# pdh930105/ARCQuant

Hardware: AMD Instinct MI355X
Metric: ARC-NVFP4 GEMM TFLOP/s (M=4096, N=KQ=4096, KE=64) (higher is better)
Workload: dtype f16

## Files before the change

### arcquant_amd/csrc/gemm_tile.hip

```cpp
#include <hip/hip_runtime.h>
#include <stdint.h>
#include <stdlib.h>

#include <type_traits>

#include "arcq_internal.hpp"
#include "gemm_common.hpp"
#include "gemm_tile_common.hpp"

namespace arcq {

#ifdef ARCQ_STREAM_STAMPS
static unsigned long long* g_tile_stamps = nullptr;
extern "C" void arcq_debug_set_tile_stamps(void* p) { g_tile_stamps = reinterpret_cast<unsigned long long*>(p); }
#define ARCQ_TILE_STAMP(k)                                                                                     \
  do {                                                                                                         \
    if (p.stamps && tid == 0) {                                                                                \
      unsigned long long t0_, t1_;                                                                             \
      asm volatile("s_memtime %0\n\ts_memrealtime %1\n\ts_waitcnt lgkmcnt(0)" : "=s"(t0_), "=s"(t1_)::"memory"); \
      p.stamps[(size_t)blockIdx.x * 4 + 2 * (k)] = t0_;                                                        \
      p.stamps[(size_t)blockIdx.x * 4 + 2 * (k) + 1] = t1_;                                                    \
    }                                                                                                          \
  } while (0)
#else
#define ARCQ_TILE_STAMP(k) do { } while (0)
#endif

template <int BM, int BN, int WAVES_M, int WAVES_N, bool kMfma32, int kEpi, bool kStagger, bool kPipe>
__global__ __launch_bounds__(WAVES_M* WAVES_N * 64) void gemm_tile_kernel(TileParams p) {
  constexpr int kThreads = WAVES_M * WAVES_N * 64;
  constexpr int WM = BM / WAVES_M, WN = BN / WAVES_N;
  constexpr int kT = kMfma32 ? 32 : 16;
  constexpr int TM = WM / kT, TN = WN / kT;
  using acc_t = typename std::conditional<kMfma32, f32x16, f32x4>::type;
  constexpr int A_UNITS = (BM * 2 + kThreads - 1) / kThreads, B_UNITS = (BN * 2 + kThreads - 1) / kThreads;
  constexpr bool A_PARTIAL = (BM * 2) % kThreads != 0, B_PARTIAL = (BN * 2) % kThreads != 0;
  static_assert(!A_PARTIAL || A_UNITS == 1, "a partial A pass is a single pass");
  static_assert(!B_PARTIAL || B_UNITS == 1, "a partial B pass is a single pass");
  constexpr int A_TILE = BM * kRowBytes, B_TILE = BN * kRowBytes;

  extern __shared__ __attribute__((aligned(16))) unsigned char smem[];
  unsigned char* const lds_a0 = smem;
  unsigned char* const lds_b0 = smem + A_TILE;
  unsigned char* const lds_a1 = smem + A_TILE + B_TILE;
  unsigned char* const lds_b1 = smem + 2 * A_TILE + B_TILE;

  const int ntiles = p.tiles_m * p.tiles_n;
  int bid = blockIdx.x, split = 0;
  if (p.splits > 1) {
    split = bid / ntiles;
    bid -= split * ntiles;
  }
  {
    const int q8 = ntiles >> 3, r8 = ntiles & 7, x = bid & 7, j = bid >> 3;
    bid = (x < r8 ? x * (q8 + 1) : r8 * (q8 + 1) + (x - r8) * q8) + j;
  }
  constexpr int kGroupM = 8;
  const int per_group = kGroupM * p.tiles_n;
  const int grp = bid / per_group;
  const int first_m = grp * kGroupM;
  const int gsz = min(p.tiles_m - first_m, kGroupM);
  const int tm = first_m + (bid % per_group) % gsz;
  const int tn = (bid % per_group) / gsz;
  const int m0 = tm * BM, n0 = tn * BN;

  const int tid = threadIdx.x;
  const int lane = tid & 63, wave = tid >> 6;
  const int wr = wave / WAVES_N, wc = wave % WAVES_N;
  const int half_k = p.K >> 1, atoms_k = p.K >> 6;
  const int a_begin = split * p.atoms_per_split, a_end = min(atoms_k, a_begin + p.atoms_per_split);

  const uint8_t* a_q[A_UNITS];
  const uint8_t* a_sf[A_UNITS];
  uint32_t a_live[A_UNITS];
  int a_slot[A_UNITS][4];
#pragma unroll
  for (int u = 0; u < A_UNITS; ++u) {
    const int unit = tid + u * kThreads, r = A_PARTIAL ? min(unit >> 1, BM - 1) : unit >> 1, h = unit & 1;
    const int row = m0 + r, rc = row < p.M ? row : p.M - 1;
    a_q[u] = p.A + (size_t)rc * half_k + h * 16;
    a_sf[u] = p.SFA + sf_atom_offset(rc, 0, atoms_k) + h * 2;
    a_live[u] = row < p.M ? 0xffffu : 0u;
#pragma unroll
    for (int j = 0; j < 4; ++j) a_slot[u][j] = kMfma32 ? lds_slot32(r, h * 4 + j) : lds_slot(r, h * 4 + j);
  }
  const uint8_t* b_q[B_UNITS];
  const uint8_t* b_sf[B_UNITS];
  uint32_t b_live[B_UNITS];
  int b_slot[B_UNITS][4];
#pragma unroll
  for (int u = 0; u < B_UNITS; ++u) {
    const int unit = tid + u * kThreads, r = B_PARTIAL ? min(unit >> 1, BN - 1) : unit >> 1, h = unit & 1;
    const int row = n0 + r, rc = row < p.N ? row : p.N - 1;
    b_q[u] = p.B + (size_t)rc * half_k + h * 16;
    b_sf[u] = p.SFB + sf_atom_offset(rc, 0, atoms_k) + h * 2;
    b_live[u] = row < p.N ? 0xffffu : 0u;
#pragma unroll
    for (int j = 0; j < 4; ++j) b_slot[u][j] = kMfma32 ? lds_slot32(r, h * 4 + j) : lds_slot(r, h * 4 + j);
  }
  const int fa_base = kMfma32 ? lds_slot32(wr * WM + (lane & 31), lane >> 5) : lds_slot(wr * WM + (lane & 15), lane >> 4);
  const int fb_base = kMfma32 ? lds_slot32(wc * WN + (lane & 31), lane >> 5) : lds_slot(wc * WN + (lane & 15), lane >> 4);
  acc_t acc[TM][TN];
#pragma unroll
  for (int i = 0; i < TM; ++i)
#pragma unroll
    for (int j = 0; j < TN; ++j)
#pragma unroll
      for (int r = 0; r < (kMfma32 ? 16 : 4); ++r) acc[i][j][r] = 0.f;

  Staged sa[A_UNITS], sb[B_UNITS];
  auto load_step = [&](int atom) {
#pragma unroll
    for (int u = 0; u < A_UNITS; ++u) sa[u] = stage_load(a_q[u], a_sf[u], atom);
#pragma unroll
    for (int u = 0; u < B_UNITS; ++u) sb[u] = stage_load(b_q[u], b_sf[u], atom);
  };
  auto store_step = [&](unsigned char* la, unsigned char* lb) {
#pragma unroll
    for (int u = 0; u < A_UNITS; ++u)
      if (!A_PARTIAL || tid < BM * 2) stage_store(la, a_slot[u], sa[u], a_live[u]);
#pragma unroll
    for (int u = 0; u < B_UNITS; ++u)
      if (!B_PARTIAL || tid < BN * 2) stage_store(lb, b_slot[u], sb[u], b_live[u]);
  };
  auto mma_step = [&](const unsigned char* la, const unsigned char* lb) {
    if constexpr (kMfma32) {
#pragma unroll
      for (int ks = 0; ks < 4; ++ks) {
        Frag8 fa[TM], fb[TN];
#pragma unroll
        for (int i = 0; i < TM; ++i) fa[i].u = *reinterpret_cast<const uint4*>(la + (fa_base ^ (ks * 32)) + i * 32 * kRowBytes);
#pragma unroll
        for (int j = 0; j < TN; ++j) fb[j].u = *reinterpret_cast<const uint4*>(lb + (fb_base ^ (ks * 32)) + j * 32 * kRowBytes);
#pragma unroll
        for (int i = 0; i < TM; ++i)
#pragma unroll
          for (int j = 0; j < TN; ++j) acc[i][j] = __builtin_amdgcn_mfma_f32_32x32x16_f16(fb[j].v, fa[i].v, acc[i][j], 0, 0, 0);
      }
    } else {
#pragma unroll
      for (int ks = 0; ks < 2; ++ks) {
        Frag8 fa[TM], fb[TN];
#pragma unroll
        for (int i = 0; i < TM; ++i) fa[i].u = *reinterpret_cast<const uint4*>(la + (fa_base ^ (ks * 64)) + i * 16 * kRowBytes);
#pragma unroll
        for (int j = 0; j < TN; ++j) fb[j].u = *reinterpret_cast<const uint4*>(lb + (fb_base ^ (ks * 64)) + j * 16 * kRowBytes);
#pragma unroll
        for (int i = 0; i < TM; ++i)
#pragma unroll
          for (int j = 0; j < TN; ++j) acc[i][j] = __builtin_amdgcn_mfma_f32_16x16x32_f16(fb[j].v, fa[i].v, acc[i][j], 0, 0, 0);
      }
    }
  };
  const bool late = kStagger && wave >= 4;
  auto k_step = [&](int kt, unsigned char* ca, unsigned char* cb, unsigned char* na, unsigned char* nb) {
    Staged ta[A_UNITS], tb[B_UNITS];
#pragma unroll
    for (int u = 0; u < A_UNITS; ++u) ta[u] = sa[u];
#pragma unroll
    for (int u = 0; u < B_UNITS; ++u) tb[u] = sb[u];
    load_step(min(kt + 2 + (late ? 1 : 0), a_end - 1));
    __builtin_amdgcn_sched_barrier(0);
    mma_step(ca, cb);
    if (kStagger && late) __syncthreads();
    unsigned char* const wa = late ? ca : na;
    unsigned char* const wb = late ? cb : nb;
#pragma unroll
    for (int u = 0; u < A_UNITS; ++u)
      if (!A_PARTIAL || tid < BM * 2) stage_store(wa, a_slot[u], ta[u], a_live[u]);
#pragma unroll
    for (int u = 0; u < B_UNITS; ++u)
      if (!B_PARTIAL || tid < BN * 2) stage_store(wb, b_slot[u], tb[u], b_live[u]);
    if (!kStagger || !late) __syncthreads();
  };

  auto k_step_pipe = [&](int kt, unsigned char* ca, unsigned char* cb, unsigned char* na, unsigned char* nb) {
    static_assert(kMfma32 || TM % 2 == 0, "pairs of A fragments");
    Staged ta[A_UNITS], tb[B_UNITS];
#pragma unroll
    for (int u = 0; u < A_UNITS; ++u) ta[u] = sa[u];
#pragma unroll
    for (int u = 0; u < B_UNITS; ++u) tb[u] = sb[u];
    load_step(min(kt + 2, a_end - 1));
    __builtin_amdgcn_sched_barrier(0);
    constexpr int kPieces = (A_UNITS + B_UNITS) * 4, kBlocks = kMfma32 ? 4 : TM;
    auto pieces = [&](int blk) {
#pragma unroll
      for (int c = blk; c < kPieces; c += kBlocks) {
        const int u = c >> 2, j = c & 3;
        if (u < A_UNITS) {
#ifdef ARCQ_EXPERIMENT_A_RAW
          if (!A_PARTIAL || tid < BM * 2) stage_piece_raw(na, a_slot[u < A_UNITS ? u : 0][j], ta[u < A_UNITS ? u : 0], a_live[u < A_UNITS ? u : 0], j);
#else
          if (!A_PARTIAL || tid < BM * 2) stage_piece(na, a_slot[u < A_UNITS ? u : 0][j], ta[u < A_UNITS ? u : 0], a_live[u < A_UNITS ? u : 0], j);
#endif
        } else {
          const int v = u - A_UNITS < B_UNITS ? u - A_UNITS : 0;
#ifdef ARCQ_EXPERIMENT_B_RAW
          if (!B_PARTIAL || tid < BN * 2) stage_piece_raw(nb, b_slot[v][j], tb[v], b_live[v], j);
#else
          if (!B_PARTIAL || tid < BN * 2) stage_piece(nb, b_slot[v][j], tb[v], b_live[v], j);
#endif
        }
      }
    };
    if constexpr (kMfma32) {
      Frag8 f32a[2][TM], f32b[2][TN];
      auto rd_set = [&](int buf, int ks) {
#pragma unroll
        for (int i = 0; i < TM; ++i) f32a[buf][i].u = *reinterpret_cast<const uint4*>(ca + (fa_base ^ (ks * 32)) + i * 32 * kRowBytes);
#pragma unroll
        for (int j = 0; j < TN; ++j) f32b[buf][j].u = *reinterpret_cast<const uint4*>(cb + (fb_base ^ (ks * 32)) + j * 32 * kRowBytes);
      };
      rd_set(0, 0);
#pragma unroll
      for (int ks = 0; ks < 4; ++ks) {
        if (ks + 1 < 4) rd_set((ks + 1) & 1, ks + 1);
        __builtin_amdgcn_sched_barrier(0);
#pragma unroll
        for (int i = 0; i < TM; ++i)
#pragma unroll
          for (int j = 0; j < TN; ++j)
            if constexpr (kMfma32)
              acc[i][j] = __builtin_amdgcn_mfma_f32_32x32x16_f16(f32b[ks & 1][j].v, f32a[ks & 1][i].v, acc[i][j], 0, 0, 0);
        pieces(ks);
        __builtin_amdgcn_sched_barrier(0);
      }
      __syncthreads();
      return;
    }
    auto rd_a = [&](int ks, int i) { Frag8 f; f.u = *reinterpret_cast<const uint4*>(ca + (fa_base ^ (ks * 64)) + i * 16 * kRowBytes); return f; };
    auto rd_b = [&](int ks, int j) { Frag8 f; f.u = *reinterpret_cast<const uint4*>(cb + (fb_base ^ (ks * 64)) + j * 16 * kRowBytes); return f; };
    constexpr int kPairs = TM / 2, kSeq = 2 * kPairs, kAhead = 1;
    Frag8 fb[2][TN], fq[kSeq][2];
    auto rd_pair = [&](int q) {
      fq[q][0] = rd_a(q / kPairs, 2 * (q % kPairs));
      fq[q][1] = rd_a(q / kPairs, 2 * (q % kPairs) + 1);
    };
#pragma unroll
    for (int j = 0; j < TN; ++j) fb[0][j] = rd_b(0, j);
#pragma unroll
    for (int q = 0; q < kAhead; ++q) rd_pair(q);
#pragma unroll
    for (int q = 0; q < kSeq; ++q) {
      const int ks = q / kPairs, pr = q % kPairs;
      if (q + kAhead < kSeq) rd_pair(q + kAhead);
      if (ks == 0 && pr == kPairs - 1 - (kAhead - 1 < kPairs - 1 ? kAhead - 1 : kPairs - 1)) {
#pragma unroll
        for (int j = 0; j < TN; ++j) fb[1][j] = rd_b(1, j);
      }
      __builtin_amdgcn_sched_barrier(0);
#pragma unroll
      for (int ii = 0; ii < 2; ++ii)
#pragma unroll
        for (int j = 0; j < TN; ++j)
          if constexpr (!kMfma32)
            acc[2 * pr + ii][j] = __builtin_amdgcn_mfma_f32_16x16x32_f16(fb[ks][j].v, fq[q][ii].v, acc[2 * pr + ii][j], 0, 0, 0);
      pieces(q);
#pragma unroll
      for (int m8 = 0; m8 < (TM == 8 ? 2 * TN : 0); ++m8) {
        __builtin_amdgcn_sched_group_barrier(0x008, 1, 0);
        __builtin_amdgcn_sched_group_barrier(0x002, 2, 0);
      }
      __builtin_amdgcn_sched_barrier(0);
    }
    __syncthreads();
  };

  load_step(a_begin);
  store_step(lds_a0, lds_b0);
  load_step(min(a_begin + 1, a_end - 1));
  if (kStagger && late) {
    store_step(lds_a1, lds_b1);
    load_step(min(a_begin + 2, a_end - 1));
  }
  __syncthreads();
  int kt = a_begin;
  if (WAVES_M * WAVES_N == 8 && wave >= 4) __builtin_amdgcn_s_setprio(1);
  ARCQ_TILE_STAMP(0);
  if constexpr (kPipe) {
    for (; kt + 1 < a_end; kt += 2) {
      k_step_pipe(kt, lds_a0, lds_b0, lds_a1, lds_b1);
      k_step_pipe(kt + 1, lds_a1, lds_b1, lds_a0, lds_b0);
    }
    if (kt < a_end) k_step_pipe(kt, lds_a0, lds_b0, lds_a1, lds_b1);
  } else {
    for (; kt + 1 < a_end; kt += 2) {
      k_step(kt, lds_a0, lds_b0, lds_a1, lds_b1);
      k_step(kt + 1, lds_a1, lds_b1, lds_a0, lds_b0);
    }
    if (kt < a_end) k_step(kt, lds_a0, lds_b0, lds_a1, lds_b1);
  }
  ARCQ_TILE_STAMP(1);

  const float alpha = p.alpha_host * (p.alpha_dev ? *p.alpha_dev : 1.0f);
  const bool vec_ok = (p.N & 3) == 0;
  uint32_t act_max = 0;
  auto store4 = [&](int m, int n, float d0, float d1, float d2, float d3, bool pre, uint2 bias2, uint2 res2) __attribute__((always_inline)) {
    if (m >= p.M || n >= p.N) return;
    const uint32_t bw[2] = {bias2.x, bias2.y}, rw[2] = {res2.x, res2.y};
    auto bias_at = [&](int r) { return bf16_bits_to_f32(pre ? (bw[r >> 1] >> (16 * (r & 1))) & 0xffffu : (uint32_t)p.bias[n + r]); };
    if (kEpi == kEpiSiluMul) {
      uint32_t y[4] = {f32_to_bf16_bits(alpha * d0), f32_to_bf16_bits(alpha * d1), f32_to_bf16_bits(alpha * d2), f32_to_bf16_bits(alpha * d3)};
      if (p.bias) {
#pragma unroll
        for (int e = 0; e < 4; ++e) y[e] = f32_to_bf16_bits(bf16_bits_to_f32(y[e]) + bias_at(e));
      }
      const uint32_t a0 = silu_mul_bf16(y[0], y[1]);
      const uint32_t a1 = silu_mul_bf16(y[2], y[3]);
      *reinterpret_cast<uint32_t*>(reinterpret_cast<uint16_t*>(p.D) + (size_t)m * (p.N >> 1) + (n >> 1)) = a0 | (a1 << 16);
      act_max = max(act_max, max(a0 & 0x7fffu, a1 & 0x7fffu));
      return;
    }
    if (p.splits > 1) {
      *reinterpret_cast<float4*>(p.partial + ((size_t)split * p.M + m) * p.N + n) = make_float4(d0, d1, d2, d3);
      return;
    }
    float d[4] = {alpha * d0, alpha * d1, alpha * d2, alpha * d3};
    if (p.bias) {
#pragma unroll
      for (int r = 0; r < 4; ++r)
        if (pre || n + r < p.N) d[r] = (p.out_dtype == ARCQ_OUT_F32 ? d[r] : bf16_bits_to_f32(f32_to_bf16_bits(d[r]))) + bias_at(r);
    }
    if (p.residual) {
#pragma unroll
      for (int r = 0; r < 4; ++r)
        if (pre || n + r < p.N) {
          const float res = bf16_bits_to_f32(pre ? (rw[r >> 1] >> (16 * (r & 1))) & 0xffffu : (uint32_t)p.residual[(size_t)m * p.N + n + r]);
          d[r] = (p.out_dtype == ARCQ_OUT_F32 ? d[r] : bf16_bits_to_f32(f32_to_bf16_bits(d[r]))) + res;
        }
    }
    if (p.out_dtype == ARCQ_OUT_F32) {
      float* o = reinterpret_cast<float*>(p.D) + (size_t)m * p.N + n;
      if (vec_ok) *reinterpret_cast<float4*>(o) = make_float4(d[0], d[1], d[2], d[3]);
      else for (int r = 0; r < 4; ++r) if (n + r < p.N) o[r] = d[r];
    } else {
      uint16_t* o = reinterpret_cast<uint16_t*>(p.D) + (size_t)m * p.N + n;
      if (vec_ok) *reinterpret_cast<uint2*>(o) = make_uint2(pack_bf16x2(d[0], d[1]), pack_bf16x2(d[2], d[3]));
      else for (int r = 0; r < 4; ++r) if (n + r < p.N) o[r] = (uint16_t)f32_to_bf16_bits(d[r]);
    }
  };
  if constexpr (kMfma32) {
#pragma unroll
    for (int i = 0; i < TM; ++i)
#pragma unroll
      for (int j = 0; j < TN; ++j) {
        const int m = m0 + wr * WM + i * 32 + (lane & 31);
#pragma unroll
        for (int g = 0; g < 4; ++g) {
          const int n = n0 + wc * WN + j * 32 + 8 * g + 4 * (lane >> 5);
          store4(m, n, acc[i][j][4 * g + 0], acc[i][j][4 * g + 1], acc[i][j][4 * g + 2], acc[i][j][4 * g + 3], false, make_uint2(0, 0), make_uint2(0, 0));
        }
      }
  } else {
    const bool pre = vec_ok && p.splits <= 1 && ((reinterpret_cast<uintptr_t>(p.bias) | reinterpret_cast<uintptr_t>(p.residual)) & 7) == 0;
    const int nb = n0 + wc * WN + 4 * (lane >> 4), mb = m0 + wr * WM + (lane & 15);
    if (pre) {
      uint2 bias_v[TN], res_cur[TN], res_nxt[TN];
#pragma unroll
      for (int j = 0; j < TN; ++j) {
        bias_v[j] = res_cur[j] = res_nxt[j] = make_uint2(0, 0);
        if (p.bias && nb + j * 16 < p.N) bias_v[j] = *reinterpret_cast<const uint2*>(p.bias + nb + j * 16);
      }
      auto res_load = [&](int i, uint2 (&r)[TN]) {
        if (!p.residual) return;
        const int m = mb + i * 16;
#pragma unroll
        for (int j = 0; j < TN; ++j)
          if (m < p.M && nb + j * 16 < p.N) r[j] = *reinterpret_cast<const uint2*>(p.residual + (size_t)m * p.N + nb + j * 16);
      };
      res_load(0, res_cur);
#pragma unroll
      for (int i = 0; i < TM; ++i) {
        if (i + 1 < TM) res_load(i + 1, res_nxt);
#pragma unroll
        for (int j = 0; j < TN; ++j) store4(mb + i * 16, nb + j * 16, acc[i][j][0], acc[i][j][1], acc[i][j][2], acc[i][j][3], true, bias_v[j], res_cur[j]);
#pragma unroll
        for (int j = 0; j < TN; ++j) res_cur[j] = res_nxt[j];
      }
    } else {
#pragma unroll
      for (int i = 0; i < TM; ++i)
#pragma unroll
        for (int j = 0; j < TN; ++j)
          store4(mb + i * 16, nb + j * 16, acc[i][j][0], acc[i][j][1], acc[i][j][2], acc[i][j][3], false, make_uint2(0, 0), make_uint2(0, 0));
    }
  }
  if (kEpi == kEpiSiluMul) {
    __shared__ uint32_t wave_max[WAVES_M * WAVES_N];
#pragma unroll
    for (int sh = 32; sh > 0; sh >>= 1) act_max = max(act_max, (uint32_t)__shfl_down((int)act_max, sh, 64));
    if (lane == 0) wave_max[wave] = act_max;
    __syncthreads();
    if (tid == 0) {
      uint32_t m = 0;
#pragma unroll
      for (int w = 0; w < WAVES_M * WAVES_N; ++w) m = max(m, wave_max[w]);
      p.slots[blockIdx.x] = m;
    }
  }
}

struct TileCfg { int id, bm, bn, waves; };
static constexpr TileCfg kTileCfgs[] = {{1, 128, 128, 4}, {2, 256, 256, 4}, {3, 256, 256, 8}, {4, 128, 256, 4}, {5, 256, 256, 8}, {6, 128, 128, 4},
                                        {7, 64, 256, 4}, {8, 32, 256, 4}, {9, 128, 128, 4}, {10, 128, 256, 8}, {11, 256, 128, 8}, {12, 128, 128, 8},
                                        {13, 64, 256, 8}, {14, 64, 128, 8}, {15, 64, 64, 4}, {16, 64, 128, 4}, {17, 128, 64, 4}};
static const TileCfg& tile_cfg(int id) {
  for (const TileCfg& c : kTileCfgs)
    if (c.id == id) return c;
  return kTileCfgs[2];
}

static int env_int(const char* name, int dflt) {
  const char* e = getenv(name);
  return e ? atoi(e) : dflt;
}
static int tile_cfg_override() {
  static const int v = env_int("ARCQ_TILE_CFG", 0);
  return v;
}
static int tile_split_override() {
  static const int v = env_int("ARCQ_TILE_SPLIT", 0);
  return v;
}
static bool tile_stagger() {
  static const int v = env_int("ARCQ_TILE_STAGGER", 0);
  return v != 0;
}
static bool tile_pipe() {
  static const int v = env_int("ARCQ_TILE_PIPE", 1);
  return v != 0;
}

static void tile_split(int64_t M, int64_t N, int64_t K, int BM, int BN, int* splits, int* atoms_per_split) {
  const int64_t tiles = ((M + BM - 1) / BM) * ((N + BN - 1) / BN);
  const int atoms = (int)(K / 64);
  int s = 1;
  if ((N % 4) == 0) {
    if (tile_split_override() > 0) s = min(tile_split_override(), max(atoms / 2, 1));
    else
      while (tiles * s < 256 && atoms / (s * 2) >= 8 && s < 32) s *= 2;
  }
  const int per = (atoms + s - 1) / s;
  *splits = (atoms + per - 1) / per;
  *atoms_per_split = per;
}

template <int BM, int BN, int WAVES_M, int WAVES_N, bool kMfma32 = false, int kEpi = kEpiPlain>
static int launch_tile(const GemmArgs& a, hipStream_t stream, bool allow_split = false) {
  TileParams p;
  p.A = a.A; p.B = a.B; p.SFA = a.SFA; p.SFB = a.SFB; p.D = a.D;
  p.alpha_dev = a.alpha_dev; p.bias = a.bias; p.residual = a.residual;
  p.M = a.M; p.N = a.N; p.K = a.K; p.alpha_host = a.alpha_host; p.out_dtype = a.out_dtype;
  p.tiles_m = (a.M + BM - 1) / BM;
  p.tiles_n = (a.N + BN - 1) / BN;
  p.splits = 1; p.atoms_per_split = a.K / 64; p.partial = nullptr;
  p.epi = a.epilogue; p.slots = a.absmax_slots;
#ifdef ARCQ_STREAM_STAMPS
  p.stamps = g_tile_stamps;
#endif
  if (allow_split && a.epilogue == kEpiPlain) {
    tile_split(a.M, a.N, a.K, BM, BN, &p.splits, &p.atoms_per_split);
    if (p.splits > 1) {
      const int64_t need = (int64_t)p.splits * a.M * a.N * (int64_t)sizeof(float);
      if (!a.workspace || a.workspace_bytes < need)
        return fail(ARCQ_ERR_WORKSPACE, "arcq_gemm_nvfp4: split-K needs %lld B of workspace, got %lld", (long long)need,
                    (long long)a.workspace_bytes);
      p.partial = reinterpret_cast<float*>(a.workspace);
    }
  }
  const size_t lds = 2 * (size_t)(BM + BN) * kRowBytes;
  constexpr bool kCanStagger = WAVES_M * WAVES_N == 8 && BM == 256 && BN == 256, kCanPipe = true;
  auto kern = gemm_tile_kernel<BM, BN, WAVES_M, WAVES_N, kMfma32, kEpi, false, false>;
  if (kCanPipe && tile_pipe()) kern = gemm_tile_kernel<BM, BN, WAVES_M, WAVES_N, kMfma32, kEpi, false, kCanPipe>;
  else if (kCanStagger && tile_stagger()) kern = gemm_tile_kernel<BM, BN, WAVES_M, WAVES_N, kMfma32, kEpi, kCanStagger, false>;
  static LdsOptIn lds_opt[3];
  const int which = (kCanPipe && tile_pipe()) ? 1 : (kCanStagger && tile_stagger()) ? 2 : 0;
  if (int rc = ensure_dynamic_lds(reinterpret_cast<const void*>(kern), lds_opt[which], (int)lds, "arcq_gemm_nvfp4 (tile)")) return rc;
  hipLaunchKernelGGL(kern, dim3((unsigned)(p.tiles_m * p.tiles_n * p.splits)), dim3(WAVES_M * WAVES_N * 64), lds, stream, p);
  hipError_t e = hipGetLastError();
  if (e != hipSuccess) return fail(ARCQ_ERR_LAUNCH, "arcq_gemm_nvfp4 (tile): launch failed: %s", hipGetErrorString(e));
  if (p.splits > 1) return gemm_splitk_finish(a, p.splits, stream);
  return ARCQ_OK;
}

static int tile_choice(int64_t M, int64_t N, int64_t K) {
  const int64_t t256 = ((M + 255) / 256) * ((N + 255) / 256);
  if (t256 >= 192) return 3;
  if (M <= 32) return 8;
  if (M <= 64) return 7;
  const int64_t t10 = ((M + 127) / 128) * ((N + 255) / 256);
  if (t10 <= 64 || t10 == 128 || (t10 > 224 && t10 <= 256) || (K >= 8192 && t10 >= 96 && t10 <= 256)) return 10;
  return 1;
}

static int effective_cfg(int64_t M, int64_t N, int64_t K, bool* may_split) {
  int id = tile_cfg_override();
  if (id == 0) id = tile_choice(M, N, K);
  id = tile_cfg(id).id;
  *may_split = !(id >= 2 && id <= 6) && id != 9;
  return id;
}

int64_t gemm_tile_silu_slots(int64_t M, int64_t N, int64_t K) {
  bool sp;
  const TileCfg& c = tile_cfg(effective_cfg(M, N, K, &sp));
  return ((M + c.bm - 1) / c.bm) * ((N + c.bn - 1) / c.bn);
}

int64_t gemm_tile_workspace_bytes(int64_t M, int64_t N, int64_t K) {
  int s = 1, per = 0;
  bool sp;
  const TileCfg& c = tile_cfg(effective_cfg(M, N, K, &sp));
  if (sp) tile_split(M, N, K, c.bm, c.bn, &s, &per);
  return s > 1 ? (int64_t)s * M * N * (int64_t)sizeof(float) : 0;
}

template <int kEpi>
static int gemm_tile_epi(const GemmArgs& a, hipStream_t stream) {
  bool sp;
  switch (effective_cfg(a.M, a.N, a.K, &sp)) {
    case 1: case 9: return launch_tile<128, 128, 2, 2, false, kEpi>(a, stream, sp);
    case 2: return launch_tile<256, 256, 2, 2, false, kEpi>(a, stream);
    case 4: return launch_tile<128, 256, 2, 2, false, kEpi>(a, stream);
    case 5: return launch_tile<256, 256, 2, 4, true, kEpi>(a, stream);
    case 6: return launch_tile<128, 128, 2, 2, true, kEpi>(a, stream);
    case 7: return launch_tile<64, 256, 1, 4, false, kEpi>(a, stream, sp);
    case 8: return launch_tile<32, 256, 1, 4, false, kEpi>(a, stream, sp);
    case 10: return launch_tile<128, 256, 2, 4, false, kEpi>(a, stream, sp);
    case 11: return launch_tile<256, 128, 4, 2, false, kEpi>(a, stream, sp);
    case 12: return launch_tile<128, 128, 2, 4, false, kEpi>(a, stream, sp);
    case 13: return launch_tile<64, 256, 1, 8, false, kEpi>(a, stream, sp);
    case 14: return launch_tile<64, 128, 2, 4, false, kEpi>(a, stream, sp);
    case 15: return launch_tile<64, 64, 2, 2, false, kEpi>(a, stream, sp);
    case 16: return launch_tile<64, 128, 2, 2, false, kEpi>(a, stream, sp);
    case 17: return launch_tile<128, 64, 2, 2, false, kEpi>(a, stream, sp);
    default: return launch_tile<256, 256, 2, 4, false, kEpi>(a, stream);
  }
}

int gemm_tile(const GemmArgs& a, hipStream_t stream) {
  return a.epilogue == kEpiSiluMul ? gemm_tile_epi<kEpiSiluMul>(a, stream) : gemm_tile_epi<kEpiPlain>(a, stream);
}

}
```

Measured before the change: 1411.

## Interleave MFMA with LDS reads and staging writes, add wide bf16 epilogue

Replaces the hard sched_barrier in the 32x32 MFMA main loop with per-MFMA sched_group_barrier groups, so LDS fragment reads, staging VALU and LDS writes are spread between matrix ops rather than bunched together. It also adds a wide epilogue that uses permlane swaps to build 16-byte bf16 stores, with bias and residual prefetched. It forces the pipelined kernel variant whenever MFMA32 is used. These aim to hide LDS latency and cut the number of store instructions, at the cost of a fragile hand-written schedule and more register pressure.

```diff
diff --git a/arcquant_amd/csrc/gemm_tile.hip b/arcquant_amd/csrc/gemm_tile.hip
--- a/arcquant_amd/csrc/gemm_tile.hip
+++ b/arcquant_amd/csrc/gemm_tile.hip
@@ -3,6 +3,7 @@
 #include <stdlib.h>
 
 #include <type_traits>
+#include <utility>
 
 #include "arcq_internal.hpp"
 #include "gemm_common.hpp"
@@ -25,6 +26,19 @@
 #else
 #define ARCQ_TILE_STAMP(k) do { } while (0)
 #endif
+
+template <int kMf, int kValu, int kRd, int kWr, int G>
+__device__ __forceinline__ void mfma_gap() {
+  __builtin_amdgcn_sched_group_barrier(0x008, 1, 0);
+  constexpr int v = kValu * (G + 1) / kMf - kValu * G / kMf;
+  if constexpr (v > 0) __builtin_amdgcn_sched_group_barrier(0x002, v, 0);
+  if constexpr (G < kRd) __builtin_amdgcn_sched_group_barrier(0x100, 1, 0);
+  if constexpr (G >= kMf - kWr) __builtin_amdgcn_sched_group_barrier(0x200, 1, 0);
+}
+template <int kMf, int kValu, int kRd, int kWr, int... G>
+__device__ __forceinline__ void mfma_gaps(std::integer_sequence<int, G...>) {
+  (mfma_gap<kMf, kValu, kRd, kWr, G>(), ...);
+}
 
 template <int BM, int BN, int WAVES_M, int WAVES_N, bool kMfma32, int kEpi, bool kStagger, bool kPipe>
 __global__ __launch_bounds__(WAVES_M* WAVES_N * 64) void gemm_tile_kernel(TileParams p) {
@@ -205,18 +219,27 @@
       }
     };
     if constexpr (kMfma32) {
+      constexpr int kMf = TM * TN, kRd = TM + TN, kWr = kPieces / kBlocks;
+      static_assert(kPieces % kBlocks == 0, "equal shares of the staging");
+      constexpr int kV = 8 * kWr, kPre = 3 * kWr;
+      constexpr bool kSpaced = kRd + kWr <= kMf;
       Frag8 f32a[2][TM], f32b[2][TN];
       auto rd_set = [&](int buf, int ks) {
 #pragma unroll
-        for (int i = 0; i < TM; ++i) f32a[buf][i].u = *reinterpret_cast<const uint4*>(ca + (fa_base ^ (ks * 32)) + i * 32 * kRowBytes);
-#pragma unroll
-        for (int j = 0; j < TN; ++j) f32b[buf][j].u = *reinterpret_cast<const uint4*>(cb + (fb_base ^ (ks * 32)) + j * 32 * kRowBytes);
+        for (int q = 0; q < kRd; ++q) {
+          if (q < 2 * TN && (q & 1) == 0) {
+            f32b[buf][q >> 1].u = *reinterpret_cast<const uint4*>(cb + (fb_base ^ (ks * 32)) + (q >> 1) * 32 * kRowBytes);
+          } else {
+            const int i = q < 2 * TN ? q >> 1 : q - TN;
+            f32a[buf][i].u = *reinterpret_cast<const uint4*>(ca + (fa_base ^ (ks * 32)) + i * 32 * kRowBytes);
+          }
+        }
       };
       rd_set(0, 0);
+      if constexpr (!kSpaced) __builtin_amdgcn_sched_barrier(0);
 #pragma unroll
       for (int ks = 0; ks < 4; ++ks) {
         if (ks + 1 < 4) rd_set((ks + 1) & 1, ks + 1);
-        __builtin_amdgcn_sched_barrier(0);
 #pragma unroll
         for (int i = 0; i < TM; ++i)
 #pragma unroll
@@ -224,6 +247,20 @@
             if constexpr (kMfma32)
               acc[i][j] = __builtin_amdgcn_mfma_f32_32x32x16_f16(f32b[ks & 1][j].v, f32a[ks & 1][i].v, acc[i][j], 0, 0, 0);
         pieces(ks);
+        if constexpr (kSpaced) {
+          constexpr auto gaps = std::make_integer_sequence<int, kMf>{};
+          if (ks == 0) {
+            __builtin_amdgcn_sched_group_barrier(0x100, kRd, 0);
+            __builtin_amdgcn_sched_group_barrier(0x002, kPre, 0);
+            mfma_gaps<kMf, kV, kRd, kWr>(gaps);
+          } else if (ks == 2) {
+            mfma_gaps<kMf, kV + 2 * kWr, kRd, kWr>(gaps);
+          } else if (ks == 1) {
+            mfma_gaps<kMf, kV, kRd, kWr>(gaps);
+          } else {
+            mfma_gaps<kMf, kV, 0, kWr>(gaps);
+          }
+        }
         __builtin_amdgcn_sched_barrier(0);
       }
       __syncthreads();
@@ -340,22 +377,161 @@
       else for (int r = 0; r < 4; ++r) if (n + r < p.N) o[r] = (uint16_t)f32_to_bf16_bits(d[r]);
     }
   };
+  auto store8 = [&](int m, int n, uint32_t (&w)[4], uint4 b, uint4 r) __attribute__((always_inline)) {
+    if (m >= p.M || n >= p.N) return;
+    if (p.bias || p.residual) {
+      const uint32_t bw[4] = {b.x, b.y, b.z, b.w}, rw[4] = {r.x, r.y, r.z, r.w};
+#pragma unroll
+      for (int e = 0; e < 4; ++e) {
+        float d2[2];
+#pragma unroll
+        for (int s = 0; s < 2; ++s) {
+          float d = bf16_bits_to_f32((w[e] >> (16 * s)) & 0xffffu);
+          if (p.bias) d = d + bf16_bits_to_f32((bw[e] >> (16 * s)) & 0xffffu);
+          if (p.residual) d = bf16_bits_to_f32(f32_to_bf16_bits(d)) + bf16_bits_to_f32((rw[e] >> (16 * s)) & 0xffffu);
+          d2[s] = d;
+        }
+        w[e] = pack_bf16x2(d2[0], d2[1]);
+      }
+    }
+    *reinterpret_cast<uint4*>(reinterpret_cast<uint16_t*>(p.D) + (size_t)m * p.N + n) = make_uint4(w[0], w[1], w[2], w[3]);
+  };
+  const uintptr_t ops = reinterpret_cast<uintptr_t>(p.bias) | reinterpret_cast<uintptr_t>(p.residual);
+  const bool pre = vec_ok && p.splits <= 1 && (ops & 7) == 0;
+  const bool wide = kEpi == kEpiPlain && pre && p.out_dtype != ARCQ_OUT_F32 && (p.N & 7) == 0 &&
+                    ((ops | reinterpret_cast<uintptr_t>(p.D)) & 15) == 0;
   if constexpr (kMfma32) {
-#pragma unroll
-    for (int i = 0; i < TM; ++i)
-#pragma unroll
-      for (int j = 0; j < TN; ++j) {
-        const int m = m0 + wr * WM + i * 32 + (lane & 31);
+    const int mb = m0 + wr * WM + (lane & 31), nb0 = n0 + wc * WN, h = lane >> 5;
+    if (wide) {
+      const int nw = nb0 + 8 * h;
+      uint4 bias_v[TN][2], res_cur[TN][2], res_nxt[TN][2];
+#pragma unroll
+      for (int j = 0; j < TN; ++j)
+#pragma unroll
+        for (int k = 0; k < 2; ++k) {
+          bias_v[j][k] = res_cur[j][k] = res_nxt[j][k] = make_uint4(0, 0, 0, 0);
+          if (p.bias && nw + 32 * j + 16 * k < p.N) bias_v[j][k] = *reinterpret_cast<const uint4*>(p.bias + nw + 32 * j + 16 * k);
+        }
+      auto res_load = [&](int i, uint4 (&r)[TN][2]) {
+        if (!p.residual) return;
+        const int m = mb + i * 32;
+#pragma unroll
+        for (int j = 0; j < TN; ++j)
+#pragma unroll
+          for (int k = 0; k < 2; ++k)
+            if (m < p.M && nw + 32 * j + 16 * k < p.N) r[j][k] = *reinterpret_cast<const uint4*>(p.residual + (size_t)m * p.N + nw + 32 * j + 16 * k);
+      };
+      res_load(0, res_cur);
+#pragma unroll
+      for (int i = 0; i < TM; ++i) {
+        if (i + 1 < TM) res_load(i + 1, res_nxt);
+        const int m = mb + i * 32;
+#pragma unroll
+        for (int j = 0; j < TN; ++j)
+#pragma unroll
+          for (int k = 0; k < 2; ++k) {
+            const acc_t& c = acc[i][j];
+            uint32_t w[4] = {pack_bf16x2(alpha * c[8 * k + 0], alpha * c[8 * k + 1]), pack_bf16x2(alpha * c[8 * k + 2], alpha * c[8 * k + 3]),
+                             pack_bf16x2(alpha * c[8 * k + 4], alpha * c[8 * k + 5]), pack_bf16x2(alpha * c[8 * k + 6], alpha * c[8 * k + 7])};
+#pragma unroll
+            for (int d = 0; d < 2; ++d) {
+              const auto r = __builtin_amdgcn_permlane32_swap(w[d], w[d + 2], false, false);
+              w[d] = r[0];
+              w[d + 2] = r[1];
+            }
+            store8(m, nw + 32 * j + 16 * k, w, bias_v[j][k], res_cur[j][k]);
+          }
+#pragma unroll
+        for (int j = 0; j < TN; ++j)
+#pragma unroll
+          for (int k = 0; k < 2; ++k) res_cur[j][k] = res_nxt[j][k];
+      }
+    } else if (pre) {
+      uint2 bias_v[TN][4], res_cur[TN][4], res_nxt[TN][4];
+#pragma unroll
+      for (int j = 0; j < TN; ++j)
 #pragma unroll
         for (int g = 0; g < 4; ++g) {
-          const int n = n0 + wc * WN + j * 32 + 8 * g + 4 * (lane >> 5);
-          store4(m, n, acc[i][j][4 * g + 0], acc[i][j][4 * g + 1], acc[i][j][4 * g + 2], acc[i][j][4 * g + 3], false, make_uint2(0, 0), make_uint2(0, 0));
+          const int n = nb0 + 32 * j + 8 * g + 4 * h;
+          bias_v[j][g] = res_cur[j][g] = res_nxt[j][g] = make_uint2(0, 0);
+          if (p.bias && n < p.N) bias_v[j][g] = *reinterpret_cast<const uint2*>(p.bias + n);
         }
-      }
+      auto res_load = [&](int i, uint2 (&r)[TN][4]) {
+        if (!p.residual) return;
+        const int m = mb + i * 32;
+#pragma unroll
+        for (int j = 0; j < TN; ++j)
+#pragma unroll
+          for (int g = 0; g < 4; ++g) {
+            const int n = nb0 + 32 * j + 8 * g + 4 * h;
+            if (m < p.M && n < p.N) r[j][g] = *reinterpret_cast<const uint2*>(p.residual + (size_t)m * p.N + n);
+          }
+      };
+      res_load(0, res_cur);
+#pragma unroll
+      for (int i = 0; i < TM; ++i) {
+        if (i + 1 < TM) res_load(i + 1, res_nxt);
+#pragma unroll
+        for (int j = 0; j < TN; ++j)
+#pragma unroll
+          for (int g = 0; g < 4; ++g)
+            store4(mb + i * 32, nb0 + 32 * j + 8 * g + 4 * h, acc[i][j][4 * g + 0], acc[i][j][4 * g + 1], acc[i][j][4 * g + 2], acc[i][j][4 * g + 3],
+                   true, bias_v[j][g], res_cur[j][g]);
+#pragma unroll
+        for (int j = 0; j < TN; ++j)
+#pragma unroll
+          for (int g = 0; g < 4; ++g) res_cur[j][g] = res_nxt[j][g];
+      }
+    } else {
+#pragma unroll
+      for (int i = 0; i < TM; ++i)
+#pragma unroll
+        for (int j = 0; j < TN; ++j)
+#pragma unroll
+          for (int g = 0; g < 4; ++g)
+            store4(mb + i * 32, nb0 + 32 * j + 8 * g + 4 * h, acc[i][j][4 * g + 0], acc[i][j][4 * g + 1], acc[i][j][4 * g + 2], acc[i][j][4 * g + 3],
+                   false, make_uint2(0, 0), make_uint2(0, 0));
+    }
   } else {
-    const bool pre = vec_ok && p.splits <= 1 && ((reinterpret_cast<uintptr_t>(p.bias) | reinterpret_cast<uintptr_t>(p.residual)) & 7) == 0;
     const int nb = n0 + wc * WN + 4 * (lane >> 4), mb = m0 + wr * WM + (lane & 15);
-    if (pre) {
+    if (TN % 2 == 0 && wide) {
+      const int g = lane >> 4, nw = n0 + wc * WN + 16 * (g & 1) + 8 * (g >> 1);
+      constexpr int TP = TN / 2 > 0 ? TN / 2 : 1;
+      uint4 bias_v[TP], res_cur[TP], res_nxt[TP];
+#pragma unroll
+      for (int jp = 0; jp < TP; ++jp) {
+        bias_v[jp] = res_cur[jp] = res_nxt[jp] = make_uint4(0, 0, 0, 0);
+        if (p.bias && nw + 32 * jp < p.N) bias_v[jp] = *reinterpret_cast<const uint4*>(p.bias + nw + 32 * jp);
+      }
+      auto res_load = [&](int i, uint4 (&r)[TP]) {
+        if (!p.residual) return;
+        const int m = mb + i * 16;
+#pragma unroll
+        for (int jp = 0; jp < TP; ++jp)
+          if (m < p.M && nw + 32 * jp < p.N) r[jp] = *reinterpret_cast<const uint4*>(p.residual + (size_t)m * p.N + nw + 32 * jp);
+      };
+      res_load(0, res_cur);
+#pragma unroll
+      for (int i = 0; i < TM; ++i) {
+        if (i + 1 < TM) res_load(i + 1, res_nxt);
+#pragma unroll
+        for (int jp = 0; jp < TP; ++jp) {
+          const acc_t& c0 = acc[i][2 * jp];
+          const acc_t& c1 = acc[i][(2 * jp + 1) % TN];
+          uint32_t w[4] = {pack_bf16x2(alpha * c0[0], alpha * c0[1]), pack_bf16x2(alpha * c0[2], alpha * c0[3]),
+                           pack_bf16x2(alpha * c1[0], alpha * c1[1]), pack_bf16x2(alpha * c1[2], alpha * c1[3])};
+#pragma unroll
+          for (int d = 0; d < 2; ++d) {
+            const auto r = __builtin_amdgcn_permlane16_swap(w[d], w[d + 2], false, false);
+            w[d] = r[0];
+            w[d + 2] = r[1];
+          }
+          store8(mb + i * 16, nw + 32 * jp, w, bias_v[jp], res_cur[jp]);
+        }
+#pragma unroll
+        for (int jp = 0; jp < TP; ++jp) res_cur[jp] = res_nxt[jp];
+      }
+    } else if (pre) {
       uint2 bias_v[TN], res_cur[TN], res_nxt[TN];
 #pragma unroll
       for (int j = 0; j < TN; ++j) {
@@ -470,12 +646,15 @@
     }
   }
   const size_t lds = 2 * (size_t)(BM + BN) * kRowBytes;
-  constexpr bool kCanStagger = WAVES_M * WAVES_N == 8 && BM == 256 && BN == 256, kCanPipe = true;
-  auto kern = gemm_tile_kernel<BM, BN, WAVES_M, WAVES_N, kMfma32, kEpi, false, false>;
-  if (kCanPipe && tile_pipe()) kern = gemm_tile_kernel<BM, BN, WAVES_M, WAVES_N, kMfma32, kEpi, false, kCanPipe>;
-  else if (kCanStagger && tile_stagger()) kern = gemm_tile_kernel<BM, BN, WAVES_M, WAVES_N, kMfma32, kEpi, kCanStagger, false>;
+  constexpr bool kCanStagger = WAVES_M * WAVES_N == 8 && BM == 256 && BN == 256 && !kMfma32, kCanPipe = true;
+  const bool pipe = kMfma32 || tile_pipe();
+  auto kern = gemm_tile_kernel<BM, BN, WAVES_M, WAVES_N, kMfma32, kEpi, false, kCanPipe>;
+  if constexpr (!kMfma32) {
+    if (!pipe) kern = gemm_tile_kernel<BM, BN, WAVES_M, WAVES_N, kMfma32, kEpi, false, false>;
+    if (!pipe && kCanStagger && tile_stagger()) kern = gemm_tile_kernel<BM, BN, WAVES_M, WAVES_N, kMfma32, kEpi, kCanStagger, false>;
+  }
   static LdsOptIn lds_opt[3];
-  const int which = (kCanPipe && tile_pipe()) ? 1 : (kCanStagger && tile_stagger()) ? 2 : 0;
+  const int which = pipe ? 1 : (kCanStagger && tile_stagger()) ? 2 : 0;
   if (int rc = ensure_dynamic_lds(reinterpret_cast<const void*>(kern), lds_opt[which], (int)lds, "arcq_gemm_nvfp4 (tile)")) return rc;
   hipLaunchKernelGGL(kern, dim3((unsigned)(p.tiles_m * p.tiles_n * p.splits)), dim3(WAVES_M * WAVES_N * 64), lds, stream, p);
   hipError_t e = hipGetLastError();
```

Measured after the change: 1429 (median of 6 runs). +1.3%, better.
